# jihun1998/AO

Hardware: AMD Instinct MI355X
Metric: points/sec fwd+bwd PTv2m2 S3DIS (higher is better)
Workload: dtype fp32

## Files before the change

ao_amd/csrc/skinny.hip:

```cpp
#include "dense_common.h"

namespace dense {

__global__ __launch_bounds__(TPB) void skinny_fwd_kernel(long long n, int cin, int cout, const float *x, const float *__restrict__ W,
                                                         const float *xsc, const float *xsh, float *y, const float *x2,
                                                         const float *xsc2, const float *xsh2, float *y2) {
    extern __shared__ float4 lds4[];
    if (blockIdx.y) { x = x2; xsc = xsc2; xsh = xsh2; y = y2; }
    float *sW = (float *)lds4;
    const int ldw = cin + 4, cq = cin >> 2;
    float *sSc = sW + (size_t)cout * ldw, *sSh = sSc + cin;
    for (int e = threadIdx.x; e < cout * cq; e += TPB) {
        const int r = e / cq, q = e - r * cq;
        *(float4 *)(sW + (size_t)r * ldw + 4 * q) = *(const float4 *)(W + (size_t)r * cin + 4 * q);
    }
    if (xsc)
        for (int e = threadIdx.x; e < cin; e += TPB) { sSc[e] = xsc[e]; sSh[e] = xsh[e]; }
    __syncthreads();
    const long long total = n * cout;
    for (long long e = (long long)blockIdx.x * TPB + threadIdx.x; e < total; e += (long long)gridDim.x * TPB) {
        const long long row = e / cout;
        const int o = (int)(e - row * cout);
        const float4 *xr = (const float4 *)(x + row * cin), *wr = (const float4 *)(sW + (size_t)o * ldw);
        float acc = 0.f;
        if (xsc) {
            int q = 0;
            for (; q + 4 <= cq; q += 4) {
                float4 av[4];
#pragma unroll
                for (int u = 0; u < 4; ++u) av[u] = xr[q + u];
#pragma unroll
                for (int u = 0; u < 4; ++u) {
                    float4 a = av[u];
                    const float4 w = wr[q + u], s4 = ((const float4 *)sSc)[q + u], h4 = ((const float4 *)sSh)[q + u];
                    a.x = fmaxf(__builtin_fmaf(a.x, s4.x, h4.x), 0.f); a.y = fmaxf(__builtin_fmaf(a.y, s4.y, h4.y), 0.f);
                    a.z = fmaxf(__builtin_fmaf(a.z, s4.z, h4.z), 0.f); a.w = fmaxf(__builtin_fmaf(a.w, s4.w, h4.w), 0.f);
                    acc = __builtin_fmaf(a.x, w.x, acc); acc = __builtin_fmaf(a.y, w.y, acc);
                    acc = __builtin_fmaf(a.z, w.z, acc); acc = __builtin_fmaf(a.w, w.w, acc);
                }
            }
            for (; q < cq; ++q) {
                float4 a = xr[q];
                const float4 w = wr[q], s4 = ((const float4 *)sSc)[q], h4 = ((const float4 *)sSh)[q];
                a.x = fmaxf(__builtin_fmaf(a.x, s4.x, h4.x), 0.f); a.y = fmaxf(__builtin_fmaf(a.y, s4.y, h4.y), 0.f);
                a.z = fmaxf(__builtin_fmaf(a.z, s4.z, h4.z), 0.f); a.w = fmaxf(__builtin_fmaf(a.w, s4.w, h4.w), 0.f);
                acc = __builtin_fmaf(a.x, w.x, acc); acc = __builtin_fmaf(a.y, w.y, acc);
                acc = __builtin_fmaf(a.z, w.z, acc); acc = __builtin_fmaf(a.w, w.w, acc);
            }
        } else {
            for (int q = 0; q < cq; ++q) {
                const float4 a = xr[q], w = wr[q];
                acc = __builtin_fmaf(a.x, w.x, acc); acc = __builtin_fmaf(a.y, w.y, acc);
                acc = __builtin_fmaf(a.z, w.z, acc); acc = __builtin_fmaf(a.w, w.w, acc);
            }
        }
        y[e] = acc;
    }
}

__global__ __launch_bounds__(TPB) void skinny_bwd_kernel(long long n, int cin, int cout, const float *gy,
                                                         const float *__restrict__ W, float *gx, const float *gy2, float *gx2,
                                                         int main_blocks, gva::PtvRiders Rs) {
    if ((int)blockIdx.x >= main_blocks) {
        if (blockIdx.y == 0) gva::rider_run(Rs, (int)blockIdx.x - main_blocks);
        return;
    }
    if (blockIdx.y) { gy = gy2; gx = gx2; }
    const int cq = cin >> 2;
    const long long total = n * cq;
    for (long long e = (long long)blockIdx.x * TPB + threadIdx.x; e < total; e += (long long)main_blocks * TPB) {
        const long long row = e / cq;
        const int q = (int)(e - row * cq);
        float4 acc = make_float4(0.f, 0.f, 0.f, 0.f);
        const float *g = gy + row * cout;
        const float *wc = W + 4 * q;
        int o = 0;
        for (; o + 6 <= cout; o += 6) {
            float sv[6];
            float4 wv[6];
#pragma unroll
            for (int u = 0; u < 6; ++u) { sv[u] = g[o + u]; wv[u] = *(const float4 *)(wc + (size_t)(o + u) * cin); }
#pragma unroll
            for (int u = 0; u < 6; ++u) {
                acc.x = __builtin_fmaf(sv[u], wv[u].x, acc.x); acc.y = __builtin_fmaf(sv[u], wv[u].y, acc.y);
                acc.z = __builtin_fmaf(sv[u], wv[u].z, acc.z); acc.w = __builtin_fmaf(sv[u], wv[u].w, acc.w);
            }
        }
        for (; o < cout; ++o) {
            const float s = g[o];
            const float4 w = *(const float4 *)(wc + (size_t)o * cin);
            acc.x = __builtin_fmaf(s, w.x, acc.x); acc.y = __builtin_fmaf(s, w.y, acc.y);
            acc.z = __builtin_fmaf(s, w.z, acc.z); acc.w = __builtin_fmaf(s, w.w, acc.w);
        }
        ((float4 *)gx)[e] = acc;
    }
}

struct SkinnyBn {
    const float *sg;
    float *gy;
    const float *x, *mean, *rstd, *gamma, *beta;
};
__global__ __launch_bounds__(TPB) void skinny_bn_bwd_reduce_kernel(int n, int c, int cout, SkinnyBn A, SkinnyBn B,
                                                                   const float *__restrict__ W, int relu, float *__restrict__ part,
                                                                   int main_blocks, gva::PtvRiders Rs) {
    extern __shared__ float4 lds4[];
    if ((int)blockIdx.x >= main_blocks) {
        if (blockIdx.y == 0) gva::rider_run(Rs, (int)blockIdx.x - main_blocks);
        return;
    }
    const SkinnyBn &S = blockIdx.y ? B : A;
    const int cq = c >> 2;
    const int rl = TPB / cq;
    const int q = threadIdx.x % cq, r = threadIdx.x / cq;
    float4 s1 = make_float4(0.f, 0.f, 0.f, 0.f), s2 = s1;
    if (r < rl) {
        const float4 m = ((const float4 *)S.mean)[q], rs = ((const float4 *)S.rstd)[q];
        const float4 g = ((const float4 *)S.gamma)[q], b = ((const float4 *)S.beta)[q];
        const float *wc = W + 4 * q;
        for (long long row = (long long)blockIdx.x * rl + r; row < n; row += (long long)main_blocks * rl) {
            const float4 v = ((const float4 *)S.x)[row * cq + q];
            const float *sg = S.sg + row * cout;
            float4 d = make_float4(0.f, 0.f, 0.f, 0.f);
            int o = 0;
            for (; o + 6 <= cout; o += 6) {
                float sv[6];
                float4 wv[6];
#pragma unroll
                for (int u = 0; u < 6; ++u) { sv[u] = sg[o + u]; wv[u] = *(const float4 *)(wc + (size_t)(o + u) * c); }
#pragma unroll
                for (int u = 0; u < 6; ++u) {
                    d.x = __builtin_fmaf(sv[u], wv[u].x, d.x); d.y = __builtin_fmaf(sv[u], wv[u].y, d.y);
                    d.z = __builtin_fmaf(sv[u], wv[u].z, d.z); d.w = __builtin_fmaf(sv[u], wv[u].w, d.w);
                }
            }
            for (; o < cout; ++o) {
                const float sv = sg[o];
                const float4 w = *(const float4 *)(wc + (size_t)o * c);
                d.x = __builtin_fmaf(sv, w.x, d.x); d.y = __builtin_fmaf(sv, w.y, d.y);
                d.z = __builtin_fmaf(sv, w.z, d.z); d.w = __builtin_fmaf(sv, w.w, d.w);
            }
            ((float4 *)S.gy)[row * cq + q] = d;
            const float4 h = bn_xhat(v, m, rs);
            if (relu) d = bn_relu_mask(d, h, g, b);
            bn_accumulate(s1, s2, d, h);
        }
    }
    column_sums_store(lds4, s1, s2, cq, rl, c, part + ((size_t)blockIdx.x * 2 + blockIdx.y) * 2 * c);
}

}

using namespace dense;

extern "C" int skinny_linear_forward_xf_hip_launcher(int n, int cin, int cout, const float *x, const float *W,
                                                    const float *xsc, const float *xsh, float *y, void *stream) {
    if (n < 0 || cin < 4 || cin % 4 != 0 || cout < 1 || cout > 64 || (xsc == nullptr) != (xsh == nullptr)) return PTV2_ERR_ARG;
    if (n == 0) return PTV2_OK;
    const size_t lds = sizeof(float) * ((size_t)cout * (cin + 4) + 2 * (size_t)cin);
    if (lds > 160 * 1024) return PTV2_ERR_ARG;
    if (lds > 32 * 1024)
        (void)hipFuncSetAttribute((const void *)skinny_fwd_kernel, hipFuncAttributeMaxDynamicSharedMemorySize, (int)lds);
    const long long total = (long long)n * cout;
    const int nblk = (int)std::min<long long>((total + TPB - 1) / TPB, 256 * 8);
    {
        PtvScopedTimer t(KID_SKINNY_FWD, (hipStream_t)stream, 4.0 * n * (cin + cout));
        hipLaunchKernelGGL(skinny_fwd_kernel, dim3(nblk), dim3(TPB), lds, (hipStream_t)stream, (long long)n, cin, cout, x, W, xsc,
                           xsh, y, (const float *)nullptr, (const float *)nullptr, (const float *)nullptr, (float *)nullptr);
    }
    PTV2_CHECK_LAUNCH();
    return PTV2_OK;
}

int skinny_linear_forward_pair(int n, int cin, int cout, const float *const *x, const float *W, const float *const *xsc,
                               const float *const *xsh, float *const *y, void *stream) {
    if (n < 0 || cin < 4 || cin % 4 != 0 || cout < 1 || cout > 64) return PTV2_ERR_ARG;
    if ((xsc[0] == nullptr) != (xsc[1] == nullptr)) return PTV2_ERR_ARG;
    if (n == 0) return PTV2_OK;
    const size_t lds = sizeof(float) * ((size_t)cout * (cin + 4) + 2 * (size_t)cin);
    if (lds > 160 * 1024) return PTV2_ERR_ARG;
    if (lds > 32 * 1024)
        (void)hipFuncSetAttribute((const void *)skinny_fwd_kernel, hipFuncAttributeMaxDynamicSharedMemorySize, (int)lds);
    const long long total = (long long)n * cout;
    const int nblk = (int)std::min<long long>((total + TPB - 1) / TPB, 256 * 8);
    {
        PtvScopedTimer t(KID_SKINNY_FWD, (hipStream_t)stream, 8.0 * n * (cin + cout));
        hipLaunchKernelGGL(skinny_fwd_kernel, dim3(nblk, 2), dim3(TPB), lds, (hipStream_t)stream, (long long)n, cin, cout, x[0], W,
                           xsc[0], xsh[0], y[0], x[1], xsc[1], xsh[1], y[1]);
    }
    PTV2_CHECK_LAUNCH();
    return PTV2_OK;
}

extern "C" int skinny_linear_forward_hip_launcher(int n, int cin, int cout, const float *x, const float *W, float *y,
                                                 void *stream) {
    return skinny_linear_forward_xf_hip_launcher(n, cin, cout, x, W, nullptr, nullptr, y, stream);
}

extern "C" int skinny_linear_backward_hip_launcher(int n, int cin, int cout, const float *gy, const float *W, float *gx,
                                                  void *stream) {
    if (n < 0 || cin < 4 || cin % 4 != 0 || cout < 1) return PTV2_ERR_ARG;
    if (n == 0) return PTV2_OK;
    const long long total = (long long)n * (cin >> 2);
    const int nblk = apply_grid(total);
    {
        PtvScopedTimer t(KID_SKINNY_BWD, (hipStream_t)stream, 4.0 * n * (cin + cout));
        hipLaunchKernelGGL(skinny_bwd_kernel, dim3(nblk), dim3(TPB), 0, (hipStream_t)stream, (long long)n, cin, cout, gy, W, gx,
                           (const float *)nullptr, (float *)nullptr, nblk, gva::PtvRiders{});
    }
    PTV2_CHECK_LAUNCH();
    return PTV2_OK;
}

int skinny_linear_backward_pair(int n, int cin, int cout, const float *const *gy, const float *W, float *const *gx, void *stream) {
    if (n < 0 || cin < 4 || cin % 4 != 0 || cout < 1) return PTV2_ERR_ARG;
    if (n == 0) return PTV2_OK;
    const long long total = (long long)n * (cin >> 2);
    const int nblk = apply_grid(total);
    {
        PtvScopedTimer t(KID_SKINNY_BWD, (hipStream_t)stream, 8.0 * n * (cin + cout));
        const gva::PtvRiders Rs = gva::ptv2_rider_take();
        hipLaunchKernelGGL(skinny_bwd_kernel, dim3(nblk + gva::rider_blocks(Rs), 2), dim3(TPB), 0, (hipStream_t)stream, (long long)n,
                           cin, cout, gy[0], W, gx[0], gy[1], gx[1], nblk, Rs);
    }
    PTV2_CHECK_LAUNCH();
    return PTV2_OK;
}

struct SkinnyBnArm {
    bool armed = false, done = false;
    int n = 0, c = 0, nblk = 0, relu = 0;
    const float *x[2] = {}, *mean[2] = {}, *rstd[2] = {}, *gamma[2] = {}, *beta[2] = {};
    const float *gy[2] = {};
    float *part = nullptr;
};
static thread_local SkinnyBnArm t_skinny_bn;

void ptv2_skinny_bn_arm(int n, int c, const float *const *x, const float *const *gy, const float *const *mean, const float *const *rstd,
                        const float *const *gamma, const float *const *beta, int relu, void *workspace, size_t workspace_bytes) {
    SkinnyBnArm &K = t_skinny_bn;
    K = SkinnyBnArm{};
    static const bool off = ptv2_env_is("AO_AMD_SKINNY_BN", '0');
    if (off || n < 1 || c < 4 || c % 4 != 0 || (c >> 2) > TPB || !workspace || workspace_bytes < dense_workspace_bytes(n, 2 * c, c)) return;
    K.armed = true;
    K.n = n; K.c = c; K.nblk = bn_grid(n, c); K.relu = relu;
    constexpr int cap = 256;
    if (n <= 16384) {
        const int rl = std::max(1, TPB / (c >> 2));
        K.nblk = (int)std::max<long long>(1, std::min<long long>(((long long)n + rl * 2 - 1) / (rl * 2), cap));
    }
    for (int i = 0; i < 2; ++i) { K.x[i] = x[i]; K.gy[i] = gy[i]; K.mean[i] = mean[i]; K.rstd[i] = rstd[i]; K.gamma[i] = gamma[i]; K.beta[i] = beta[i]; }
    K.part = (float *)workspace;
}
void ptv2_skinny_bn_disarm(void) { t_skinny_bn.armed = false; }

int skinny_backward_pair_bn_reduce(int n, int cin, int cout, const float *const *gy, const float *W, float *const *gx, void *stream) {
    SkinnyBnArm &K = t_skinny_bn;
    const bool fuse = K.armed && K.n == n && K.c == cin && K.gy[0] == gx[0] && K.gy[1] == gx[1] && n > 0;
    K.armed = false;
    if (!fuse) return skinny_linear_backward_pair(n, cin, cout, gy, W, gx, stream);
    hipStream_t st = (hipStream_t)stream;
    {
        PtvScopedTimer t(KID_SKINNY_BWD, st, 8.0 * n * (cin + cout) + 8.0 * n * cin);
        const gva::PtvRiders Rs = gva::ptv2_rider_take();
        const SkinnyBn A{gy[0], gx[0], K.x[0], K.mean[0], K.rstd[0], K.gamma[0], K.beta[0]};
        const SkinnyBn B{gy[1], gx[1], K.x[1], K.mean[1], K.rstd[1], K.gamma[1], K.beta[1]};
        hipLaunchKernelGGL(skinny_bn_bwd_reduce_kernel, dim3(K.nblk + gva::rider_blocks(Rs), 2), dim3(TPB), sizeof(float4) * 2 * TPB, st,
                           n, cin, cout, A, B, W, K.relu, K.part, K.nblk, Rs);
    }
    K.done = true;
    PTV2_CHECK_LAUNCH();
    return PTV2_OK;
}

int ptv2_skinny_bn_take_records(int n, int c, const float *part, const float *const *gy) {
    SkinnyBnArm &K = t_skinny_bn;
    const bool reduced = K.done && K.part == part && K.n == n && K.c == c && K.gy[0] == gy[0] && K.gy[1] == gy[1];
    K.done = false;
    return reduced ? K.nblk : 0;
}
```

Measured before the change: 12.85 million.

## Tile skinny linear forward through LDS and stage BN-backward weights and grads

New measurement: 12.99 million, median of 6. +1.1%, better.

```diff
diff --git a/ao_amd/csrc/skinny.hip b/ao_amd/csrc/skinny.hip
--- a/ao_amd/csrc/skinny.hip
+++ b/ao_amd/csrc/skinny.hip
@@ -55,6 +55,84 @@
             }
         }
         y[e] = acc;
+    }
+}
+
+__device__ __forceinline__ void stage_rows4(float4 *dst, const float4 *__restrict__ src, int total, int cq, int ld4) {
+    for (int b = 0; b < total; b += 8 * TPB) {
+        float4 v[8];
+        int e[8];
+#pragma unroll
+        for (int u = 0; u < 8; ++u) {
+            e[u] = min(b + u * TPB + (int)threadIdx.x, total - 1);
+            v[u] = src[e[u]];
+        }
+        __builtin_amdgcn_sched_barrier(0);
+#pragma unroll
+        for (int u = 0; u < 8; ++u) dst[(e[u] / cq) * ld4 + e[u] % cq] = v[u];
+    }
+}
+
+constexpr int SKINNY_TILE_LOADS = 4;
+static inline int skinny_tile_rows(int cin) { return SKINNY_TILE_LOADS * TPB / (cin >> 2); }
+
+template <bool XF>
+__global__ __launch_bounds__(TPB) void skinny_fwd_tile_kernel(int n, int cin, int cout, int R, int ntiles, const float *x,
+                                                              const float *__restrict__ W, const float *xsc, const float *xsh,
+                                                              float *y, const float *x2, const float *xsc2, const float *xsh2,
+                                                              float *y2) {
+    extern __shared__ float4 lds4[];
+    if (blockIdx.y) { x = x2; xsc = xsc2; xsh = xsh2; y = y2; }
+    const int cq = cin >> 2, ld4 = cq + 1, te = R * cq;
+    float4 *sW = lds4, *sX = lds4 + (size_t)cout * ld4;
+    int tr[SKINNY_TILE_LOADS], tq[SKINNY_TILE_LOADS];
+    float4 xv[SKINNY_TILE_LOADS], s4[SKINNY_TILE_LOADS], h4[SKINNY_TILE_LOADS];
+#pragma unroll
+    for (int u = 0; u < SKINNY_TILE_LOADS; ++u) {
+        const int e = min((int)threadIdx.x + u * TPB, te - 1);
+        tr[u] = e / cq;
+        tq[u] = e - tr[u] * cq;
+    }
+    long long tile = blockIdx.x;
+#pragma unroll
+    for (int u = 0; u < SKINNY_TILE_LOADS; ++u) {
+        const long long row = min(tile * R + tr[u], (long long)n - 1);
+        xv[u] = ((const float4 *)x)[row * cq + tq[u]];
+        if (XF) { s4[u] = ((const float4 *)xsc)[tq[u]]; h4[u] = ((const float4 *)xsh)[tq[u]]; }
+    }
+    stage_rows4(sW, (const float4 *)W, cout * cq, cq, ld4);
+    const int outs = R * cout;
+    for (; tile < ntiles; tile += gridDim.x) {
+#pragma unroll
+        for (int u = 0; u < SKINNY_TILE_LOADS; ++u) {
+            float4 a = xv[u];
+            if (XF) {
+                a.x = fmaxf(__builtin_fmaf(a.x, s4[u].x, h4[u].x), 0.f); a.y = fmaxf(__builtin_fmaf(a.y, s4[u].y, h4[u].y), 0.f);
+                a.z = fmaxf(__builtin_fmaf(a.z, s4[u].z, h4[u].z), 0.f); a.w = fmaxf(__builtin_fmaf(a.w, s4[u].w, h4[u].w), 0.f);
+            }
+            sX[tr[u] * ld4 + tq[u]] = a;
+        }
+        __syncthreads();
+        const long long next = tile + gridDim.x;
+#pragma unroll
+        for (int u = 0; u < SKINNY_TILE_LOADS; ++u) {
+            const long long row = min(next * R + tr[u], (long long)n - 1);
+            xv[u] = ((const float4 *)x)[row * cq + tq[u]];
+        }
+        for (int e = threadIdx.x; e < outs; e += TPB) {
+            const int r = e / cout, o = e - r * cout;
+            const float4 *xr = sX + r * ld4, *wr = sW + o * ld4;
+            float acc = 0.f;
+#pragma unroll 4
+            for (int q = 0; q < cq; ++q) {
+                const float4 a = xr[q], w = wr[q];
+                acc = __builtin_fmaf(a.x, w.x, acc); acc = __builtin_fmaf(a.y, w.y, acc);
+                acc = __builtin_fmaf(a.z, w.z, acc); acc = __builtin_fmaf(a.w, w.w, acc);
+            }
+            const long long row = tile * R + r;
+            if (row < n) y[row * cout + o] = acc;
+        }
+        __syncthreads();
     }
 }
 
@@ -149,25 +227,118 @@
     column_sums_store(lds4, s1, s2, cq, rl, c, part + ((size_t)blockIdx.x * 2 + blockIdx.y) * 2 * c);
 }
 
+constexpr int SKINNY_BN_TRIP = 4, SKINNY_BN_SG = 2;
+__global__ __launch_bounds__(TPB) void skinny_bn_bwd_reduce_staged_kernel(int n, int c, int cout, SkinnyBn A, SkinnyBn B,
+                                                                          const float *__restrict__ W, int relu,
+                                                                          float *__restrict__ part, int main_blocks, gva::PtvRiders Rs) {
+    extern __shared__ float4 lds4[];
+    if ((int)blockIdx.x >= main_blocks) {
+        if (blockIdx.y == 0) gva::rider_run(Rs, (int)blockIdx.x - main_blocks);
+        return;
+    }
+    const SkinnyBn &S = blockIdx.y ? B : A;
+    const int cq = c >> 2;
+    const int rl = TPB / cq;
+    const int q = threadIdx.x % cq, r = threadIdx.x / cq;
+    const int rg = rl * cout, ng = SKINNY_BN_TRIP * rg;
+    float *sG = (float *)(lds4 + (size_t)cout * cq);
+    const long long step = (long long)main_blocks * rl, last = (long long)n * cout - 1;
+    const float4 m = ((const float4 *)S.mean)[q], rs = ((const float4 *)S.rstd)[q];
+    const float4 g = ((const float4 *)S.gamma)[q], b = ((const float4 *)S.beta)[q];
+    int ge[SKINNY_BN_SG], gu[SKINNY_BN_SG], gw[SKINNY_BN_SG];
+#pragma unroll
+    for (int j = 0; j < SKINNY_BN_SG; ++j) {
+        ge[j] = min((int)threadIdx.x + j * TPB, ng - 1);
+        gu[j] = ge[j] / rg;
+        gw[j] = ge[j] - gu[j] * rg;
+    }
+    float4 v[SKINNY_BN_TRIP], s1 = make_float4(0.f, 0.f, 0.f, 0.f), s2 = s1;
+    float gs[SKINNY_BN_SG];
+    long long b0 = (long long)blockIdx.x * rl;
+#define SKINNY_BN_LOADS(base)                                                                                          \
+    _Pragma("unroll") for (int u = 0; u < SKINNY_BN_TRIP; ++u)                                                         \
+        v[u] = ((const float4 *)S.x)[min((base) + u * step + r, (long long)n - 1) * cq + q];                           \
+    _Pragma("unroll") for (int j = 0; j < SKINNY_BN_SG; ++j) gs[j] = S.sg[min(((base) + gu[j] * step) * cout + gw[j], last)];
+    SKINNY_BN_LOADS(b0)
+    if (b0 < n) stage_rows4(lds4, (const float4 *)W, cout * cq, cq, cq);
+    const float *sg = sG + min(r, rl - 1) * cout;
+    const float4 *wq = lds4 + q;
+    for (; b0 < n; b0 += SKINNY_BN_TRIP * step) {
+        float4 vc[SKINNY_BN_TRIP], d[SKINNY_BN_TRIP];
+#pragma unroll
+        for (int u = 0; u < SKINNY_BN_TRIP; ++u) { vc[u] = v[u]; d[u] = make_float4(0.f, 0.f, 0.f, 0.f); }
+#pragma unroll
+        for (int j = 0; j < SKINNY_BN_SG; ++j) sG[ge[j]] = gs[j];
+        __syncthreads();
+        SKINNY_BN_LOADS(b0 + SKINNY_BN_TRIP * step)
+#pragma unroll 12
+        for (int o = 0; o < cout; ++o) {
+            const float4 w = wq[(size_t)o * cq];
+#pragma unroll
+            for (int u = 0; u < SKINNY_BN_TRIP; ++u) {
+                const float sv = sg[u * rg + o];
+                d[u].x = __builtin_fmaf(sv, w.x, d[u].x); d[u].y = __builtin_fmaf(sv, w.y, d[u].y);
+                d[u].z = __builtin_fmaf(sv, w.z, d[u].z); d[u].w = __builtin_fmaf(sv, w.w, d[u].w);
+            }
+        }
+#pragma unroll
+        for (int u = 0; u < SKINNY_BN_TRIP; ++u) {
+            const long long row = b0 + u * step + r;
+            if (r < rl && row < n) {
+                ((float4 *)S.gy)[row * cq + q] = d[u];
+                const float4 h = bn_xhat(vc[u], m, rs);
+                if (relu) d[u] = bn_relu_mask(d[u], h, g, b);
+                bn_accumulate(s1, s2, d[u], h);
+            }
+        }
+        __syncthreads();
+    }
+#undef SKINNY_BN_LOADS
+    column_sums_store(lds4, s1, s2, cq, rl, c, part + ((size_t)blockIdx.x * 2 + blockIdx.y) * 2 * c);
+}
+
 }
 
 using namespace dense;
 
-extern "C" int skinny_linear_forward_xf_hip_launcher(int n, int cin, int cout, const float *x, const float *W,
-                                                    const float *xsc, const float *xsh, float *y, void *stream) {
-    if (n < 0 || cin < 4 || cin % 4 != 0 || cout < 1 || cout > 64 || (xsc == nullptr) != (xsh == nullptr)) return PTV2_ERR_ARG;
-    if (n == 0) return PTV2_OK;
+static inline bool skinny_lanes_only() { return ptv2_env_is("AO_AMD_SKINNY", 'l'); }
+
+static int skinny_forward_run(int n, int cin, int cout, int sets, const float *const *x, const float *W, const float *const *xsc,
+                              const float *const *xsh, float *const *y, hipStream_t st) {
+    const int R = skinny_tile_rows(cin);
+    const size_t tile_lds = sizeof(float) * (size_t)(cout + R) * (cin + 4);
+    const bool tile = !skinny_lanes_only() && R >= 1 && tile_lds <= 160 * 1024;
+    const float *x1 = sets > 1 ? x[1] : nullptr, *sc1 = sets > 1 ? xsc[1] : nullptr, *sh1 = sets > 1 ? xsh[1] : nullptr;
+    float *y1 = sets > 1 ? y[1] : nullptr;
+    PtvScopedTimer t(KID_SKINNY_FWD, st, 4.0 * sets * n * (cin + cout));
+    if (tile) {
+        const int per_cu = (int)std::max<size_t>(1, std::min<size_t>(4, 160 * 1024 / tile_lds));
+        const int ntiles = (n + R - 1) / R, cap = std::max(1, 256 * per_cu / sets);
+        const int walk = (ntiles + cap - 1) / cap, nblk = (ntiles + walk - 1) / walk;
+        auto kernel = xsc[0] ? skinny_fwd_tile_kernel<true> : skinny_fwd_tile_kernel<false>;
+        if (tile_lds > 32 * 1024)
+            (void)hipFuncSetAttribute((const void *)kernel, hipFuncAttributeMaxDynamicSharedMemorySize, (int)tile_lds);
+        hipLaunchKernelGGL(kernel, dim3(nblk, sets), dim3(TPB), tile_lds, st, n, cin, cout, R, ntiles, x[0], W, xsc[0], xsh[0], y[0],
+                           x1, sc1, sh1, y1);
+        return PTV2_OK;
+    }
     const size_t lds = sizeof(float) * ((size_t)cout * (cin + 4) + 2 * (size_t)cin);
     if (lds > 160 * 1024) return PTV2_ERR_ARG;
     if (lds > 32 * 1024)
         (void)hipFuncSetAttribute((const void *)skinny_fwd_kernel, hipFuncAttributeMaxDynamicSharedMemorySize, (int)lds);
     const long long total = (long long)n * cout;
     const int nblk = (int)std::min<long long>((total + TPB - 1) / TPB, 256 * 8);
-    {
-        PtvScopedTimer t(KID_SKINNY_FWD, (hipStream_t)stream, 4.0 * n * (cin + cout));
-        hipLaunchKernelGGL(skinny_fwd_kernel, dim3(nblk), dim3(TPB), lds, (hipStream_t)stream, (long long)n, cin, cout, x, W, xsc,
-                           xsh, y, (const float *)nullptr, (const float *)nullptr, (const float *)nullptr, (float *)nullptr);
-    }
+    hipLaunchKernelGGL(skinny_fwd_kernel, dim3(nblk, sets), dim3(TPB), lds, st, (long long)n, cin, cout, x[0], W, xsc[0], xsh[0], y[0],
+                       x1, sc1, sh1, y1);
+    return PTV2_OK;
+}
+
+extern "C" int skinny_linear_forward_xf_hip_launcher(int n, int cin, int cout, const float *x, const float *W,
+                                                    const float *xsc, const float *xsh, float *y, void *stream) {
+    if (n < 0 || cin < 4 || cin % 4 != 0 || cout < 1 || cout > 64 || (xsc == nullptr) != (xsh == nullptr)) return PTV2_ERR_ARG;
+    if (n == 0) return PTV2_OK;
+    if (sizeof(float) * ((size_t)cout * (cin + 4) + 2 * (size_t)cin) > 160 * 1024) return PTV2_ERR_ARG;
+    RUN(skinny_forward_run(n, cin, cout, 1, &x, W, &xsc, &xsh, &y, (hipStream_t)stream));
     PTV2_CHECK_LAUNCH();
     return PTV2_OK;
 }
@@ -177,17 +348,8 @@
     if (n < 0 || cin < 4 || cin % 4 != 0 || cout < 1 || cout > 64) return PTV2_ERR_ARG;
     if ((xsc[0] == nullptr) != (xsc[1] == nullptr)) return PTV2_ERR_ARG;
     if (n == 0) return PTV2_OK;
-    const size_t lds = sizeof(float) * ((size_t)cout * (cin + 4) + 2 * (size_t)cin);
-    if (lds > 160 * 1024) return PTV2_ERR_ARG;
-    if (lds > 32 * 1024)
-        (void)hipFuncSetAttribute((const void *)skinny_fwd_kernel, hipFuncAttributeMaxDynamicSharedMemorySize, (int)lds);
-    const long long total = (long long)n * cout;
-    const int nblk = (int)std::min<long long>((total + TPB - 1) / TPB, 256 * 8);
-    {
-        PtvScopedTimer t(KID_SKINNY_FWD, (hipStream_t)stream, 8.0 * n * (cin + cout));
-        hipLaunchKernelGGL(skinny_fwd_kernel, dim3(nblk, 2), dim3(TPB), lds, (hipStream_t)stream, (long long)n, cin, cout, x[0], W,
-                           xsc[0], xsh[0], y[0], x[1], xsc[1], xsh[1], y[1]);
-    }
+    if (sizeof(float) * ((size_t)cout * (cin + 4) + 2 * (size_t)cin) > 160 * 1024) return PTV2_ERR_ARG;
+    RUN(skinny_forward_run(n, cin, cout, 2, x, W, xsc, xsh, y, (hipStream_t)stream));
     PTV2_CHECK_LAUNCH();
     return PTV2_OK;
 }
@@ -265,8 +427,12 @@
         const gva::PtvRiders Rs = gva::ptv2_rider_take();
         const SkinnyBn A{gy[0], gx[0], K.x[0], K.mean[0], K.rstd[0], K.gamma[0], K.beta[0]};
         const SkinnyBn B{gy[1], gx[1], K.x[1], K.mean[1], K.rstd[1], K.gamma[1], K.beta[1]};
-        hipLaunchKernelGGL(skinny_bn_bwd_reduce_kernel, dim3(K.nblk + gva::rider_blocks(Rs), 2), dim3(TPB), sizeof(float4) * 2 * TPB, st,
-                           n, cin, cout, A, B, W, K.relu, K.part, K.nblk, Rs);
+        const size_t rec_lds = sizeof(float4) * 2 * TPB;
+        const size_t sg_lds = sizeof(float) * SKINNY_BN_TRIP * (TPB / (cin >> 2)) * cout, w_lds = sizeof(float) * (size_t)cout * cin;
+        const bool staged = !skinny_lanes_only() && sg_lds <= sizeof(float) * SKINNY_BN_SG * TPB && w_lds + sg_lds <= 28 * 1024;
+        hipLaunchKernelGGL(staged ? skinny_bn_bwd_reduce_staged_kernel : skinny_bn_bwd_reduce_kernel,
+                           dim3(K.nblk + gva::rider_blocks(Rs), 2), dim3(TPB), staged ? std::max(rec_lds, w_lds + sg_lds) : rec_lds, st, n,
+                           cin, cout, A, B, W, K.relu, K.part, K.nblk, Rs);
     }
     K.done = true;
     PTV2_CHECK_LAUNCH();
```
